# 0411tony/Yue

Hardware: AMD Instinct MI355X
Metric: BPR triplet-updates/sec at k=128 (S-round semantics, user rows sequential; the reference's exact sequential semantics: secondary.exact) (higher is better)
Workload: dtype f32

## Files before the change

yue_amd/csrc/bpr_host.hip:

```cpp
#include "host_common.hpp"

#include "train_kernels.hpp"
#include "round_kernels.hpp"

using yue_host::fail;
using yue_host::kr_of;
using yue_host::with_kr;
static_assert(yue::kNllSlots == yue_host::kNllSlotsHost && yue::kHeaderSlack == yue_host::kHeaderSlackHost &&
              yue::kMetaStageMax == (uint32_t)yue_host::kMetaStageMaxHost, "host_common.hpp mirrors these");

namespace {

yue::TrainArgs make_args(yue_ctx *c, double lr, double regU, double regI) {
    yue::TrainArgs a{};
    a.P = c->P.p; a.Q = c->Q.p; a.dP = c->dP.p; a.dQ = c->dQ.p;
    a.stage = c->Q.p ? c->Q.p + (size_t)c->n * c->k : nullptr;
    a.ev_u = c->ev_u.p; a.ev_i = c->ev_i.p; a.ev_j = c->ev_j.p;
    a.indptr = c->indptr.p; a.indices = c->indices.p;
    a.nll_slots = c->scal.p;
    a.m = c->m; a.n = c->n; a.k = c->k;
    a.lr = lr;
    a.ru = (float)(lr * regU);
    a.ri = (float)(lr * regI);
    a.neg_lo = 0; a.neg_range = (int32_t)c->n;
// ... 351 lines not shown
    if (!c || !c->have_factors) return fail(YUE_ERR_ARG, "yue_bpr_replay: no factors uploaded");
    if (T < 0 || (T > 0 && (!u || !i || !j))) return fail(YUE_ERR_ARG, "yue_bpr_replay: bad triplet arrays");
    HIPCHK(hipSetDevice(c->device));
    if (!c->opt_replay_levels) {
        int rc = upload_triplets(c, u, i, j, T, false);
        if (rc) return rc;
        if ((rc = zero_scalars(c))) return rc;
        if ((rc = yue_host::chain_stream(c, T, lr, regU, regI))) return rc;
        return read_scalars(c, nll_out, nullptr, nullptr);
    }
    std::vector<int32_t> lastP((size_t)c->m, 0), lastQ((size_t)c->n, 0), lvl((size_t)T);
    int32_t nlev = 0;
    for (int64_t t = 0; t < T; ++t) {
        if (u[t] < 0 || u[t] >= c->m || i[t] < 0 || i[t] >= c->n || j[t] >= c->n) return fail(YUE_ERR_ARG, "triplet " + std::to_string(t) + " out of range");
        if (j[t] < 0) { lvl[(size_t)t] = 0; continue; }
        if (i[t] == j[t]) return fail(YUE_ERR_ARG, "triplet " + std::to_string(t) + ": i == j");
        int32_t l = std::max(lastP[(size_t)u[t]], std::max(lastQ[(size_t)i[t]], lastQ[(size_t)j[t]])) + 1;
        lvl[(size_t)t] = l;
        lastP[(size_t)u[t]] = lastQ[(size_t)i[t]] = lastQ[(size_t)j[t]] = l;
        nlev = std::max(nlev, l);
    }
    std::vector<int64_t> lptr((size_t)nlev + 2, 0);
    for (int64_t t = 0; t < T; ++t) if (lvl[(size_t)t] > 0) lptr[(size_t)lvl[(size_t)t] + 1]++;
    for (int32_t l = 1; l <= nlev; ++l) lptr[(size_t)l + 1] += lptr[(size_t)l];
    const int64_t Tv = lptr[(size_t)nlev + 1];
    std::vector<int32_t> pu((size_t)std::max<int64_t>(Tv, 1)), pi((size_t)std::max<int64_t>(Tv, 1)), pj((size_t)std::max<int64_t>(Tv, 1));
    {
        std::vector<int64_t> cur(lptr.begin(), lptr.end());
        for (int64_t t = 0; t < T; ++t) {
            const int32_t l = lvl[(size_t)t];
            if (l == 0) continue;
            const int64_t o = cur[(size_t)l]++;
            pu[(size_t)o] = u[t]; pi[(size_t)o] = i[t]; pj[(size_t)o] = j[t];
        }
    }
    int rc = upload_triplets(c, pu.data(), pi.data(), pj.data(), Tv, true);
    if (rc) return rc;
    yue::TrainArgs a = make_args(c, lr, regU, regI);
    a.ev_u = c->xu.p; a.ev_i = c->xi.p; a.ev_j = c->xj.p;
    if ((rc = zero_scalars(c))) return rc;
    c->replay_levels = nlev;
    for (int32_t l = 1; l <= nlev; ++l) {
        const int64_t e0 = lptr[(size_t)l], e1 = lptr[(size_t)l + 1];
        if (e1 > e0) launch_level(c, a, e0, e1);
    }
    HIPCHK(hipGetLastError());
    return read_scalars(c, nll_out, nullptr, nullptr);
}

int yue_bpr_rounds(yue_ctx *c, const int32_t *u, const int32_t *i, const int32_t *j, const int64_t *round_ptr, int64_t n_rounds,
                   double lr, double regU, double regI, double *nll_out) {
    if (!c || !c->have_factors) return fail(YUE_ERR_ARG, "yue_bpr_rounds: no factors uploaded");
    if (!round_ptr || n_rounds < 0) return fail(YUE_ERR_ARG, "yue_bpr_rounds: bad round_ptr");
    HIPCHK(hipSetDevice(c->device));
    const int64_t T = round_ptr[n_rounds];
    if (round_ptr[0] != 0) return fail(YUE_ERR_ARG, "yue_bpr_rounds: round_ptr[0] must be 0");
    for (int64_t r = 0; r < n_rounds; ++r) if (round_ptr[r + 1] < round_ptr[r]) return fail(YUE_ERR_ARG, "yue_bpr_rounds: round_ptr must be non-decreasing");
    if (c->m * (int64_t)c->k * 4 >= (1ll << 31)) {
        const int tpw = tpw_of(c, false);
        for (int64_t r = 0; r < n_rounds; ++r)
            for (int64_t b = round_ptr[r]; b < round_ptr[r + 1]; b += tpw) {
                int32_t lo = u[b], hi = u[b];
                for (int64_t t = b; t < std::min(round_ptr[r + 1], b + tpw); ++t) { lo = std::min(lo, u[t]); hi = std::max(hi, u[t]); }
                if ((int64_t)(hi - lo) * c->k * 4 >= (1ll << 31)) return fail(YUE_ERR_ARG, "yue_bpr_rounds: users of neighbouring triplets are more than 2 GiB of factor rows apart; group the triplets by user");
            }
    }
    int rc = upload_triplets(c, u, i, j, T, true);
    if (rc) return rc;
    yue::TrainArgs a = make_args(c, lr, regU, regI);
    a.ev_u = c->xu.p; a.ev_i = c->xi.p; a.ev_j = c->xj.p;
    if ((rc = zero_scalars(c))) return rc;
    std::vector<int64_t> bounds(round_ptr, round_ptr + n_rounds + 1);
    if ((rc = run_rounds(c, a, bounds, 1, [](int64_t) { return YUE_OK; }))) { reset_round_state(c); return rc; }
    HIPCHK(hipGetLastError());
    return read_scalars(c, nll_out, nullptr, nullptr);
}

int yue_cune_steps(yue_ctx *c, const int32_t *u, const int32_t *i, const int32_t *k, const int32_t *j, int64_t T,
                   double s, double lr, double regU, double regI, double *loss_out) {
    if (!c || !c->have_factors) return fail(YUE_ERR_ARG, "yue_cune_steps: no factors uploaded");
    if (T < 0 || (T > 0 && (!u || !i || !k || !j || !loss_out)) || !(s > 0.0)) return fail(YUE_ERR_ARG, "yue_cune_steps: bad argument");
    if (T == 0) return YUE_OK;
    HIPCHK(hipSetDevice(c->device));
    for (int64_t t = 0; t < T; ++t) {
        if (u[t] < 0 || u[t] >= c->m || i[t] < 0 || i[t] >= c->n || j[t] < 0 || j[t] >= c->n || k[t] >= c->n) return fail(YUE_ERR_ARG, "yue_cune_steps: step " + std::to_string(t) + " out of range");
        if (i[t] == j[t] || k[t] == i[t]) return fail(YUE_ERR_ARG, "yue_cune_steps: step " + std::to_string(t) + ": i must differ from k and from j (k == j is allowed, as in the reference)");
    }
    int rc = upload_triplets(c, u, i, j, T, true);
    if (rc) return rc;
    HIPCHK(c->xk.resize(T)); HIPCHK(c->x_loss.resize(T));
    HIPCHK(hipMemcpyAsync(c->xk.p, k, T * sizeof(int32_t), hipMemcpyHostToDevice, c->stream));
    yue::CuneArgs a{};
    a.P = c->P.p; a.Q = c->Q.p; a.k = c->k; a.u = c->xu.p; a.i = c->xi.p; a.kk = c->xk.p; a.j = c->xj.p; a.T = T;
    a.inv_s = 1.0 / s; a.inv_s32 = (float)(1.0 / s); a.lr = lr;
    a.ru = (float)(lr * regU); a.ri = (float)(lr * regI);
    a.loss_out = c->x_loss.p;
    with_kr(c->k, [&](auto kr) { hipLaunchKernelGGL(yue::k_cune_steps<kr()>, dim3(1), dim3(64), 0, c->stream, a); });
    HIPCHK(hipGetLastError());
    HIPCHK(hipMemcpyAsync(loss_out, c->x_loss.p, T * sizeof(double), hipMemcpyDeviceToHost, c->stream));
    HIPCHK(hipStreamSynchronize(c->stream));
    return YUE_OK;
}

int yue_adam_reset(yue_ctx *c) {
    if (!c || !c->have_factors) return fail(YUE_ERR_ARG, "yue_adam_reset: no factors uploaded");
    HIPCHK(hipSetDevice(c->device));
    const size_t mk = (size_t)c->m * c->k, nk = (size_t)c->n * c->k;
    HIPCHK(c->aU_m.resize(mk)); HIPCHK(c->aU_v.resize(mk)); HIPCHK(c->aV_m.resize(nk)); HIPCHK(c->aV_v.resize(nk));
    HIPCHK(hipMemsetAsync(c->aU_m.p, 0, mk * sizeof(float), c->stream)); HIPCHK(hipMemsetAsync(c->aU_v.p, 0, mk * sizeof(float), c->stream));
    HIPCHK(hipMemsetAsync(c->aV_m.p, 0, nk * sizeof(float), c->stream)); HIPCHK(hipMemsetAsync(c->aV_v.p, 0, nk * sizeof(float), c->stream));
    HIPCHK(hipMemsetAsync(c->dP.p, 0, mk * sizeof(float), c->stream)); HIPCHK(hipMemsetAsync(c->dQ.p, 0, nk * sizeof(float), c->stream));
    c->adam_m = c->m; c->adam_n = c->n; c->adam_k = c->k;
    return YUE_OK;
}

int yue_adam_get_moments(yue_ctx *c, float *mU, float *vU, float *mV, float *vV) {
    if (!c || !c->have_factors || c->adam_m != c->m || c->adam_n != c->n || c->adam_k != c->k)
        return fail(YUE_ERR_ARG, "yue_adam_get_moments: no Adam state for the uploaded factors");
    HIPCHK(hipSetDevice(c->device));
    HIPCHK(hipStreamSynchronize(c->stream));
    const size_t mk = (size_t)c->m * c->k * sizeof(float), nk = (size_t)c->n * c->k * sizeof(float);
    if (mU) HIPCHK(hipMemcpy(mU, c->aU_m.p, mk, hipMemcpyDeviceToHost));
    if (vU) HIPCHK(hipMemcpy(vU, c->aU_v.p, mk, hipMemcpyDeviceToHost));
    if (mV) HIPCHK(hipMemcpy(mV, c->aV_m.p, nk, hipMemcpyDeviceToHost));
    if (vV) HIPCHK(hipMemcpy(vV, c->aV_v.p, nk, hipMemcpyDeviceToHost));
    return YUE_OK;
}

int yue_adam_step(yue_ctx *c, const int32_t *u, const int32_t *i, const int32_t *j, int64_t T, double lr, double reg, int64_t step, double *loss_out) {
    if (!c || !c->have_factors) return fail(YUE_ERR_ARG, "yue_adam_step: no factors uploaded");
    if (T <= 0 || !u || !i || !j || step < 1) return fail(YUE_ERR_ARG, "yue_adam_step: bad argument (T > 0, step >= 1)");
    HIPCHK(hipSetDevice(c->device));
    if (c->adam_m != c->m || c->adam_n != c->n || c->adam_k != c->k) { const int rc0 = yue_adam_reset(c); if (rc0) return rc0; }
    for (int64_t t = 0; t < T; ++t)
        if (u[t] < 0 || u[t] >= c->m || i[t] < 0 || i[t] >= c->n || j[t] < 0 || j[t] >= c->n) return fail(YUE_ERR_ARG, "yue_adam_step: triplet " + std::to_string(t) + " out of range");
    int rc = upload_triplets(c, u, i, j, T, true);
    if (rc) return rc;
    if ((rc = zero_scalars(c))) return rc;
    yue::MbArgs a{};
    a.U = c->P.p; a.V = c->Q.p; a.gU = c->dP.p; a.gV = c->dQ.p; a.k = c->k; a.u = c->xu.p; a.i = c->xi.p; a.j = c->xj.p; a.T = T;
    a.reg = (float)reg; a.loss_slots = c->scal.p;
    const dim3 grid((unsigned)(((T + 31) / 32 + 3) / 4));
    with_kr(c->k, [&](auto kr) { hipLaunchKernelGGL(yue::k_mb_grad<kr()>, grid, dim3(256), 0, c->stream, a); });
    if ((rc = yue_host::adam_apply(c, lr, step))) return rc;
    return read_scalars(c, loss_out, nullptr, nullptr);
}

int yue_sample_negatives(yue_ctx *c, uint64_t seed, uint32_t epoch, int32_t *j_out) {
    if (!c || !c->have_inter || !j_out) return fail(YUE_ERR_ARG, "yue_sample_negatives: no interactions uploaded");
    HIPCHK(hipSetDevice(c->device));
    yue::TrainArgs a = make_args(c, 0, 0, 0);
    a.seed = seed; a.epoch = epoch;
    if (c->E > 0) {
        hipLaunchKernelGGL(yue::k_sample, dim3((unsigned)((c->E + 255) / 256)), dim3(256), 0, c->stream, a, c->E);
        HIPCHK(hipGetLastError());
        HIPCHK(hipMemcpyAsync(j_out, c->ev_j.p, c->E * sizeof(int32_t), hipMemcpyDeviceToHost, c->stream));
    }
    HIPCHK(hipStreamSynchronize(c->stream));
    return YUE_OK;
}

int yue_sumsq(yue_ctx *c, double *sp, double *sq) {
    if (!c || !c->have_factors) return fail(YUE_ERR_ARG, "yue_sumsq: no factors uploaded");
    HIPCHK(hipSetDevice(c->device));
    int rc = sumsq_async(c);
    if (rc) return rc;
    double h[2];
    HIPCHK(hipMemcpyAsync(h, c->scal.p + yue::kNllSlots + 1, sizeof h, hipMemcpyDeviceToHost, c->stream));
    HIPCHK(hipStreamSynchronize(c->stream));
    if (sp) *sp = h[0];
    if (sq) *sq = h[1];
    return YUE_OK;
}

int yue_bpr_epoch(yue_ctx *c, uint64_t seed, uint32_t epoch, int64_t round_events, double lr, double regU, double regI,
                  double *nll_out, double *sumsqP_out, double *sumsqQ_out) {
    if (!c || !c->have_factors || !c->have_inter) return fail(YUE_ERR_ARG, "yue_bpr_epoch: upload factors and interactions first");
    if (round_events < 0) return fail(YUE_ERR_ARG, "yue_bpr_epoch: round_events must be positive (or 0 for the device's default)");
    HIPCHK(hipSetDevice(c->device));
    yue::TrainArgs a = make_args(c, lr, regU, regI);
    a.seed = seed + 0x632BE59BD9B4E019ull * (uint64_t)c->rank;
    a.epoch = epoch;
    int rc = zero_scalars(c);
    if (rc) return rc;
    const int64_t E = c->E;
    if (E > 0) hipLaunchKernelGGL(yue::k_sample, dim3((unsigned)((E + 255) / 256)), dim3(256), 0, c->stream, a, E);
    if (c->opt_epoch_exact) {
        if (yue_host::on_communicator(c) && c->nranks > 1) return fail(YUE_ERR_ARG, "yue_bpr_epoch: option epoch_exact runs on one GPU (the sequential order spans all item shards)");
        if ((rc = yue_host::chain_epoch(c, lr, regU, regI))) return rc;
        if ((rc = sumsq_async(c))) return rc;
        return read_scalars(c, nll_out, sumsqP_out, sumsqQ_out);
    }
    std::vector<int64_t> bounds;
    double tot[2] = {(double)E, (double)c->n};
    if (yue_host::on_communicator(c)) {
        if ((rc = yue_allreduce_f64(c, tot, 2))) return rc;
        if ((rc = zero_scalars(c))) return rc;
    }
    const double etot = tot[0];
    if (round_events == 0 && (rc = default_round_events(c, tot[1] / c->nranks, &round_events))) return rc;
    int64_t ub = 1, group = 1;
    if ((rc = yue_epoch_plan(c->m, c->k, round_events, etot, c->nranks, &ub, &group, nullptr))) return rc;
    if (!yue_host::on_communicator(c)) group = std::max<int64_t>(1, (c->m + ub - 1) / ub);
    else group = std::max<int64_t>(1, ((int64_t)c->opt_comm_group_mb << 20) / std::max<int64_t>(1, ub * c->k * 4));
    std::vector<int64_t> ublock;
    for (int64_t u0 = 0; u0 < c->m; u0 += ub) { ublock.push_back(u0); bounds.push_back(c->h_ev_ptr[(size_t)u0]); }
    ublock.push_back(c->m); bounds.push_back(E);
    const int64_t R = (int64_t)ublock.size() - 1;
    const bool seq_user = !yue_host::on_communicator(c) && c->opt_round_user_seq && meta_path_fits(c);
    if (seq_user) {
        HIPCHK(c->d_ev_ptr.resize((size_t)c->m + 1));
        if (!c->d_ev_ptr_valid) {
            HIPCHK(hipMemcpyAsync(c->d_ev_ptr.p, c->h_ev_ptr.data(), ((size_t)c->m + 1) * sizeof(int64_t), hipMemcpyHostToDevice, c->stream));
            c->d_ev_ptr_valid = true;
        }
        HIPCHK(c->margins.resize((size_t)std::max<int64_t>(E, 1)));
    }
    c->psq_in_rounds = seq_user && c->all_users_have_events && E > 0;
    if (c->psq_in_rounds) {
        HIPCHK(c->psq_slots.resize((size_t)yue::kNllSlots));
        HIPCHK(hipMemsetAsync(c->psq_slots.p, 0, (size_t)yue::kNllSlots * sizeof(double), c->stream));
    }
    c->last_round_user_seq = 0;
    auto after = [&](int64_t r) -> int {
        if (seq_user && !c->bigq) { c->last_round_user_seq = 1; return YUE_OK; }
        if ((r + 1) % group != 0 && r + 1 != R) return YUE_OK;
        const int64_t g_first = ublock[(size_t)(r - (r % group))], g_last = ublock[(size_t)r + 1];
        const int64_t first = g_first * c->k, count = (g_last - g_first) * c->k;
        const dim3 grid((unsigned)std::min<int64_t>(4096, (count + 255) / 256));
        if (!yue_host::on_communicator(c)) {
            hipLaunchKernelGGL(yue::k_apply_range, grid, dim3(256), 0, c->stream, c->P.p, c->dP.p, first, count);
            return YUE_OK;
        }
        HIPCHK(hipEventRecord(c->ev_rounds, c->stream));
        HIPCHK(hipStreamWaitEvent(c->comm_stream, c->ev_rounds, 0));
        c->comm_collectives += 1;
        c->comm_bytes += (double)count * sizeof(float);
        if (const int rcr = yue_host::reduce_user_block(c, first, count, c->comm_stream)) return rcr;
        hipLaunchKernelGGL(yue::k_apply_range, grid, dim3(256), 0, c->comm_stream, c->P.p, c->dP.p, first, count);
        return YUE_OK;
    };
    c->comm_collectives = 0; c->comm_bytes = 0.0; c->comm_wait_ms = 0.0;
    if ((rc = run_rounds(c, a, bounds, 0, after, meta_path_fits(c), seq_user ? &ublock : nullptr))) { reset_round_state(c); return rc; }
    if (c->last_round_user_seq && E > 0)
        hipLaunchKernelGGL(yue::k_loss_margins, dim3(2048), dim3(256), 0, c->stream, c->margins.p, c->ev_j.p, E, c->scal.p);
    const bool psq_done = c->psq_in_rounds && c->last_round_user_seq;
    c->psq_in_rounds = false;
    if (yue_host::on_communicator(c)) {
        HIPCHK(hipEventRecord(c->ev_t_rounds, c->stream));
        HIPCHK(hipEventRecord(c->ev_t_comm, c->comm_stream));
    }
    HIPCHK(hipEventRecord(c->ev_comm, c->comm_stream));
    HIPCHK(hipStreamWaitEvent(c->stream, c->ev_comm, 0));
    c->comm_compute_waits = 1;
    HIPCHK(hipGetLastError());
    if ((rc = sumsq_async(c, psq_done ? c->psq_slots.p : nullptr))) return rc;
    if ((rc = read_scalars(c, nll_out, sumsqP_out, sumsqQ_out))) return rc;
    if (yue_host::on_communicator(c)) {
        float ms = 0.f;
        HIPCHK(hipEventSynchronize(c->ev_t_comm));
        HIPCHK(hipEventElapsedTime(&ms, c->ev_t_rounds, c->ev_t_comm));
        c->comm_wait_ms = ms > 0.f ? ms : 0.0;
    }
    return YUE_OK;
}

int yue_epoch_plan(int64_t m, int k, int64_t round_events, double events_total, int nranks,
                   int64_t *user_block, int64_t *blocks_per_group, int64_t *n_blocks) {
    if (m <= 0 || k <= 0 || round_events <= 0 || nranks < 1 || !(events_total >= 0.0)) return fail(YUE_ERR_ARG, "yue_epoch_plan: bad argument");
    const double per_user = events_total / (double)nranks / (double)m;
    const int64_t ub = std::max<int64_t>(1, (int64_t)std::floor((double)round_events / std::max(per_user, 1e-9) + 0.5));
    if (user_block) *user_block = ub;
    if (blocks_per_group) *blocks_per_group = std::max<int64_t>(1, (8ll << 20) / std::max<int64_t>(1, ub * k * 4));
    if (n_blocks) *n_blocks = (m + ub - 1) / ub;
    return YUE_OK;
}

int yue_default_round_events(yue_ctx *c, int64_t *out) {
    if (!c || !c->have_factors || !out) return fail(YUE_ERR_ARG, "yue_default_round_events: upload factors first (the value depends on k)");
    HIPCHK(hipSetDevice(c->device));
    double n_rows = (double)c->n;
    if (yue_host::on_communicator(c)) {
        const int rc = yue_allreduce_f64(c, &n_rows, 1);
        if (rc) return rc;
        n_rows /= c->nranks;
    }
    return default_round_events(c, n_rows, out);
}

int yue_set_kernel_timing(yue_ctx *c, int stride) {
    if (!c || stride < 0) return fail(YUE_ERR_ARG, "yue_set_kernel_timing: bad argument");
    c->timing_stride = stride;
    c->ev_used = 0;
    return YUE_OK;
}

int yue_get_kernel_timing(yue_ctx *c, double *total_ms, int64_t *launches, int64_t *triplets) {
    if (!c) return fail(YUE_ERR_ARG, "null context");
    HIPCHK(hipSetDevice(c->device));
    HIPCHK(hipStreamSynchronize(c->stream));
    double tot = 0.0;
    int64_t trip = 0, nl = 0;
    for (size_t t = 0; t < c->ev_used; ++t) {
        float ms = 0.f;
        HIPCHK(hipEventElapsedTime(&ms, c->ev_pool[t].first, c->ev_pool[t].second));
        tot += ms;
        trip += c->ev_triplets[t];
        nl += c->ev_launches[t];
    }
    if (total_ms) *total_ms = tot;
    if (launches) *launches = nl;
    if (triplets) *triplets = trip;
    c->ev_used = 0;
    return YUE_OK;
}

#ifdef YUE_STAMPS
int yue_debug_get_stamps(yue_ctx *c, unsigned long long *out, int64_t max_waves, int64_t *n_waves) {
    HIPCHK(hipStreamSynchronize(c->stream));
    const int64_t w = std::min(max_waves, c->stamp_waves);
    if (w > 0) HIPCHK(hipMemcpy(out, c->stamps.p, (size_t)w * 64, hipMemcpyDeviceToHost));
    *n_waves = w;
    return YUE_OK;
}
#endif

}
```

yue_amd/csrc/round_kernels.hpp:

```cpp
#pragma once
#include "train_kernels.hpp"

#ifdef YUE_ABL_NO_HOT
#define YUE_M_HOT(val, rs, vo, so) asm volatile("" :: "v"(val))
#else
#define YUE_M_HOT(val, rs, vo, so) YUE_BATOMIC(val, rs, vo, so)
#endif
#ifdef YUE_ABL_NO_DP
#define YUE_M_DP(val, rs, vo, so) asm volatile("" :: "v"(val))
#else
#define YUE_M_DP(val, rs, vo, so) YUE_BATOMIC(val, rs, vo, so)
#endif

#define YUE_BLOAD_NT(rs, vo, so) __builtin_bit_cast(float, __builtin_amdgcn_raw_buffer_load_b32((rs), (vo), (so), 2))
#if defined(YUE_EXP_LOAD_CACHED)
#define YUE_M_LOAD_J(rs, vo, so) YUE_BLOAD(rs, vo, so)
#define YUE_M_LOAD_I(rs, vo, so) YUE_BLOAD(rs, vo, so)
#elif defined(YUE_EXP_LOAD_NT)
#define YUE_M_LOAD_J(rs, vo, so) YUE_BLOAD_NT(rs, vo, so)
#define YUE_M_LOAD_I(rs, vo, so) YUE_BLOAD_NT(rs, vo, so)
#else
#define YUE_M_LOAD_J(rs, vo, so) YUE_BLOAD_NT(rs, vo, so)
#define YUE_M_LOAD_I(rs, vo, so) YUE_BLOAD(rs, vo, so)
#endif
// ... 347 lines not shown
                    }
                }
            } else {
            if (!hot_i) {
#pragma unroll
                for (int r = 0; r < KR; ++r) YUE_BSTORE(full_i ? o[r].qi2 : o[r].qi2 - qi[t][r], rsQ, vo[r], wi);
            } else {
#pragma unroll
                for (int r = 0; r < KR; ++r) YUE_M_HOT(o[r].qi2 - qi[t][r], rsdQ, vo[r], oi[t]);
            }
            if (!hot_j) {
#pragma unroll
                for (int r = 0; r < KR; ++r) YUE_BSTORE(full_j ? o[r].qj2 : o[r].qj2 - qj[t][r], rsQ, vo[r], wj);
            } else {
#pragma unroll
                for (int r = 0; r < KR; ++r) YUE_M_HOT(o[r].qj2 - qj[t][r], rsdQ, vo[r], oj[t]);
            }
            }
        }
        const bool exists = base + t < ra.e_end;
        const bool last = exists && ((t == TPW - 1) || base + t + 1 >= ra.e_end || ru_[t + 1 < TPW ? t + 1 : t] != ru_[t]);
        if (last) {
            if (run_ok) {
#pragma unroll
                for (int r = 0; r < KR; ++r) YUE_M_DP(dp[r], rsdP, vo[r], ou[t]);
            }
#pragma unroll
            for (int r = 0; r < KR; ++r) dp[r] = 0.0f;
            run_ok = false;
        }
        __builtin_amdgcn_sched_barrier(0);
    }
    YUE_STAMP(4, ""); YUE_STAMP(5, ""); YUE_STAMP(6, "");
#pragma unroll
    for (int off = 1; off < TPW; off <<= 1) nll += __shfl_xor(nll, off);
    if (lane == 0 && nll != 0.0) atomicAdd(a.nll_slots + (wave & (kNllSlots - 1)), nll);
    YUE_STAMP(7, "s_waitcnt vmcnt(0)");
}

struct RoundUArgs {
    int64_t u_begin, u_end;
    const int64_t *ev_ptr;
    int64_t e_begin, e_end;
    int staged;
    float *margins;
    double *psq_slots;
};

template <int KR, bool FAST>
__global__ void __launch_bounds__(256) k_round_u(TrainArgs a, RoundUArgs ra, const int32_t *__restrict__ evi, const int32_t *__restrict__ evj,
                                                 const uint32_t *__restrict__ mti, const uint32_t *__restrict__ mtj) {
    const int lane = threadIdx.x & 63;
    const int64_t wave = (int64_t)blockIdx.x * 4 + __builtin_amdgcn_readfirstlane((int)(threadIdx.x >> 6));
    const int64_t u = ra.u_begin + wave;
    if (u >= ra.u_end) return;
    const int64_t e0 = ra.ev_ptr[u], e1 = ra.ev_ptr[u + 1];
    if (e1 <= e0) return;
    const unsigned k = (unsigned)a.k;
    const unsigned row_bytes = k * 4u;
    unsigned vo[KR];
#pragma unroll
    for (int r = 0; r < KR; ++r) { const unsigned e = 64u * r + lane; vo[r] = e < k ? e * 4u : kOobOffset; }
    const uint64_t qbytes = (uint64_t)a.n * row_bytes;
    const int qrec = (int)(qbytes < 0x7fffffffull ? qbytes : 0x7fffffffull);
    const unsigned stage0 = (unsigned)a.n * row_bytes;
    const uint64_t qsbytes = qbytes + (ra.staged ? 2ull * (uint64_t)(ra.e_end - ra.e_begin) * row_bytes : 0ull);
    const int qsrec = (int)(qsbytes < 0x7fffffffull ? qsbytes : 0x7fffffffull);
    const auto rsQ = __builtin_amdgcn_make_buffer_rsrc(a.Q, 0, qsrec, kRsrcFlags);
    const auto rsdQ = __builtin_amdgcn_make_buffer_rsrc(a.dQ, 0, qrec, kRsrcFlags);
    float *prow = a.P + (uint64_t)u * k;
    float p[KR];
#pragma unroll
    for (int r = 0; r < KR; ++r) { const unsigned e = 64u * r + lane; p[r] = e < k ? prow[e] : 0.0f; }
    const float lrf = (float)a.lr;
    const unsigned len = (unsigned)(e1 - e0 < 0x7fffffff ? e1 - e0 : 0x7fffffff);
    for (unsigned seg = 0; seg < len; seg += 64u) {
        int hI, hJ;
        uint32_t hMI, hMJ;
        {
            const bool ex = seg + (unsigned)lane < len;
            const int64_t e = e0 + seg + (ex ? lane : 0);
            hI = evi[e]; hJ = evj[e]; hMI = mti[e]; hMJ = mtj[e];
            if (!ex) { hI = 0; hJ = -1; hMI = 0u; hMJ = 0u; }
        }
        const unsigned seg_len = len - seg < 64u ? len - seg : 64u;
        float xs = 0.0f;
        auto gather = [&](float (&qi)[KR], float (&qj)[KR], unsigned t) {
            const int ti = __builtin_amdgcn_readlane(hI, t), tj = __builtin_amdgcn_readlane(hJ, t);
            const unsigned oi = (unsigned)ti * row_bytes, oj = (unsigned)(tj < 0 ? 0 : tj) * row_bytes;
#pragma unroll
            for (int r = 0; r < KR; ++r) { qi[r] = YUE_M_LOAD_I(rsQ, vo[r], oi); qj[r] = YUE_M_LOAD_J(rsQ, vo[r], oj); }
        };
        auto step = [&](const float (&qi)[KR], const float (&qj)[KR], unsigned t) {
            const int tj = __builtin_amdgcn_readlane(hJ, t);
            if (tj < 0) return;
            const int ti = __builtin_amdgcn_readlane(hI, t);
            const uint32_t mi = (uint32_t)__builtin_amdgcn_readlane((int)hMI, t), mj = (uint32_t)__builtin_amdgcn_readlane((int)hMJ, t);
            float ai = 0.0f, aj = 0.0f;
#pragma unroll
            for (int r = 0; r < KR; ++r) { const float a1 = p[r] * qi[r]; ai = ai + a1; const float a2 = p[r] * qj[r]; aj = aj + a2; }
            const float x = wave_sum(ai) - wave_sum(aj);
            const float c = FAST ? chain_coef_fast(x, lrf) : (float)(a.lr * (1.0 - chain_sigmoid(x)));
            xs = (unsigned)lane == t ? x : xs;
            const unsigned cli = meta_kind(mi), clj = meta_kind(mj);
            const bool uniq_i = cli == kMetaUnique, uniq_j = clj == kMetaUnique;
            const bool full_i = uniq_i || meta_first(mi), full_j = uniq_j || meta_first(mj);
            const unsigned oi = (unsigned)ti * row_bytes, oj = (unsigned)tj * row_bytes;
            const unsigned wi = uniq_i ? oi : stage0 + meta_slot(mi) * row_bytes;
            const unsigned wj = uniq_j ? oj : stage0 + meta_slot(mj) * row_bytes;
            Elem o[KR];
#pragma unroll
            for (int r = 0; r < KR; ++r) { o[r] = bpr_elem(p[r], qi[r], qj[r], c, a.ru, a.ri); p[r] = o[r].p2; }
            if (cli != kMetaHot) {
#pragma unroll
                for (int r = 0; r < KR; ++r) YUE_BSTORE(full_i ? o[r].qi2 : o[r].qi2 - qi[r], rsQ, vo[r], wi);
            } else {
#pragma unroll
                for (int r = 0; r < KR; ++r) YUE_M_HOT(o[r].qi2 - qi[r], rsdQ, vo[r], oi);
            }
            if (clj != kMetaHot) {
#pragma unroll
                for (int r = 0; r < KR; ++r) YUE_BSTORE(full_j ? o[r].qj2 : o[r].qj2 - qj[r], rsQ, vo[r], wj);
            } else {
#pragma unroll
                for (int r = 0; r < KR; ++r) YUE_M_HOT(o[r].qj2 - qj[r], rsdQ, vo[r], oj);
            }
        };
        constexpr int D = KR == 1 ? 8 : 4;
        float qi[D][KR], qj[D][KR];
#pragma unroll
        for (int s_ = 0; s_ < D; ++s_) gather(qi[s_], qj[s_], (unsigned)s_);
        for (unsigned t = 0; t < seg_len; t += D) {
#pragma unroll
            for (int s_ = 0; s_ < D; ++s_) {
                step(qi[s_], qj[s_], t + s_);
                gather(qi[s_], qj[s_], (t + s_ + D) & 63u);
            }
        }
        if ((unsigned)lane < seg_len) ra.margins[e0 + seg + lane] = xs;
    }
#pragma unroll
    for (int r = 0; r < KR; ++r) { const unsigned e = 64u * r + lane; if (e < k) prow[e] = p[r]; }
    if (ra.psq_slots) {
        double s = 0.0;
#pragma unroll
        for (int r = 0; r < KR; ++r) { const unsigned e = 64u * r + lane; const float sq = p[r] * p[r]; if (e < k) s += (double)sq; }
#pragma unroll
        for (int off = 1; off < 64; off <<= 1) s += __shfl_xor(s, off);
        if (lane == 0) atomicAdd(ra.psq_slots + (u & (kNllSlots - 1)), s);
    }
}

__global__ void __launch_bounds__(256) k_loss_margins(const float *__restrict__ x, const int32_t *__restrict__ evj, int64_t E, double *nll_slots) {
    double nl = 0.0;
    const int64_t stride = (int64_t)gridDim.x * blockDim.x;
    for (int64_t e = (int64_t)blockIdx.x * blockDim.x + threadIdx.x; e < E; e += stride)
        if (evj[e] >= 0) nl += -log(chain_sigmoid(x[e]));
#pragma unroll
    for (int off = 1; off < 64; off <<= 1) nl += __shfl_xor(nl, off);
    if ((threadIdx.x & 63) == 0 && nl != 0.0) atomicAdd(nll_slots + ((blockIdx.x * 4 + (threadIdx.x >> 6)) & (kNllSlots - 1)), nl);
}

struct FoldArgs {
    const uint2 *fold;
    const unsigned long long *round_rows;
    float *Q, *dQ;
    const float *stage;
    int k;
    uint32_t capacity;
};

template <int KR, int EPG>
__device__ __forceinline__ void fold_group(const FoldArgs &f, int lane, unsigned k, uint32_t nact, const uint2 (&ent)[4]) {
    float st[EPG][4][KR];
    unsigned el[KR];
    bool big = false;
#pragma unroll
    for (int r = 0; r < KR; ++r) el[r] = min(64u * r + lane, k - 1u);
#pragma unroll
    for (int sl = 0; sl < EPG; ++sl) {
        if ((uint32_t)sl >= nact) continue;
        const uint32_t c = fold_count(ent[sl].y);
        const bool hot = c == 0u;
        const float *src = hot ? f.dQ + (uint64_t)ent[sl].x * k : f.stage + (uint64_t)fold_block(ent[sl].y) * k;
#pragma unroll
        for (int r = 0; r < KR; ++r) st[sl][0][r] = YUE_FOLD_LD(src + el[r]);
        if (hot) {
            const float *row = f.Q + (uint64_t)ent[sl].x * k;
#pragma unroll
            for (int r = 0; r < KR; ++r) st[sl][1][r] = YUE_FOLD_LDROW(row + el[r]);
        } else {
#pragma unroll
            for (int r = 0; r < KR; ++r) st[sl][1][r] = YUE_FOLD_LD(src + (uint64_t)k + el[r]);
        }
        if (c > 2u) {
#pragma unroll
            for (unsigned q = 2; q < 4; ++q)
#pragma unroll
                for (int r = 0; r < KR; ++r) st[sl][q][r] = YUE_FOLD_LD(src + (uint64_t)(q < c ? q : 0u) * k + el[r]);
        }
        big = big || c > 4u;
    }
#pragma unroll
    for (int sl = 0; sl < EPG; ++sl) {
        if ((uint32_t)sl >= nact) continue;
        const uint32_t c = fold_count(ent[sl].y);
        const bool hot = c == 0u;
        float *row = f.Q + (uint64_t)ent[sl].x * k;
        float *dr = f.dQ + (uint64_t)ent[sl].x * k;
#pragma unroll
        for (int r = 0; r < KR; ++r) {
            const unsigned e = 64u * r + lane;
            float acc = st[sl][1][r];
#pragma unroll
            for (unsigned q = 2; q < 4; ++q) { const float v = q < c ? st[sl][q][r] : 0.0f; acc = acc + v; }
            st[sl][1][r] = acc;
            if (c <= 4u && e < k) {
                row[e] = st[sl][0][r] + acc;
                if (hot) dr[e] = 0.0f;
            }
        }
    }
    if (big) {
#pragma unroll
        for (int sl = 0; sl < EPG; ++sl) {
            if ((uint32_t)sl >= nact) continue;
            const uint32_t c = fold_count(ent[sl].y);
            if (c <= 4u) continue;
            const float *src = f.stage + (uint64_t)fold_block(ent[sl].y) * k;
            float *row = f.Q + (uint64_t)ent[sl].x * k;
            float acc[KR];
#pragma unroll
            for (int r = 0; r < KR; ++r) acc[r] = st[sl][1][r];
            constexpr unsigned STEP = KR == 1 ? 8u : 4u;
            for (uint32_t q0 = 4u; q0 < c; q0 += STEP) {
                float v[STEP][KR];
#pragma unroll
                for (unsigned q = 0; q < STEP; ++q)
#pragma unroll
                    for (int r = 0; r < KR; ++r) v[q][r] = YUE_FOLD_LD(src + (uint64_t)(q0 + q < c ? q0 + q : q0) * k + el[r]);
#pragma unroll
                for (unsigned q = 0; q < STEP; ++q)
#pragma unroll
                    for (int r = 0; r < KR; ++r) acc[r] = acc[r] + (q0 + q < c ? v[q][r] : 0.0f);
            }
#pragma unroll
            for (int r = 0; r < KR; ++r) { const unsigned e = 64u * r + lane; if (e < k) row[e] = st[sl][0][r] + acc[r]; }
        }
    }
}

template <int KR>
__global__ void __launch_bounds__(256) k_round_fold(FoldArgs f) {
    constexpr int EPG = KR == 4 ? 2 : 4;
    const int lane = threadIdx.x & 63;
    const uint32_t wave = blockIdx.x * 4u + (uint32_t)__builtin_amdgcn_readfirstlane((int)(threadIdx.x >> 6));
    const uint32_t nwaves = gridDim.x * 4u;
    const unsigned k = (unsigned)f.k;
    const uint32_t b0 = wave * EPG;
    uint2 ent[4];
    typedef uint32_t u32x8 __attribute__((ext_vector_type(8)));
    u32x8 ev;
    unsigned long long cntw;
    const bool spec = b0 + 4u <= f.capacity;
    const uint2 *first = f.fold + (spec ? b0 : 0u);
    asm volatile("s_load_dwordx8 %0, %2, 0x0\n\ts_load_dwordx2 %1, %3, 0x0\n\ts_waitcnt lgkmcnt(0)"
                 : "=&s"(ev), "=&s"(cntw) : "s"(first), "s"(f.round_rows) : "memory");
    const uint32_t cnt = (uint32_t)(cntw >> 32);
    ent[0] = make_uint2(ev[0], ev[1]); ent[1] = make_uint2(ev[2], ev[3]); ent[2] = make_uint2(ev[4], ev[5]); ent[3] = make_uint2(ev[6], ev[7]);
    if (b0 < cnt) {
        if (!spec) {
#pragma unroll
            for (int sl = 0; sl < EPG; ++sl) ent[sl] = f.fold[b0 + sl < cnt ? b0 + sl : b0];
        }
        fold_group<KR, EPG>(f, lane, k, min((uint32_t)EPG, cnt - b0), ent);
    }
    for (uint32_t b = b0 + nwaves * EPG; b < cnt; b += nwaves * EPG) {
#pragma unroll
        for (int sl = 0; sl < EPG; ++sl) ent[sl] = f.fold[b + sl < cnt ? b + sl : b];
        fold_group<KR, EPG>(f, lane, k, min((uint32_t)EPG, cnt - b), ent);
    }
}

}
```

yue_amd/csrc/train_kernels.hpp:

```cpp
#pragma once
#include "bpr_device.hpp"

namespace yue {

__global__ void __launch_bounds__(256) k_sample(TrainArgs a, int64_t E) {
    int64_t e = (int64_t)blockIdx.x * blockDim.x + threadIdx.x;
    if (e < E) a.ev_j[e] = sample_negative(a, a.ev_u[e], e);
}

template <int KR>
__global__ void __launch_bounds__(256) k_bpr_level(TrainArgs a, int64_t e_begin, int64_t e_end, int tpw) {
    const int lane = threadIdx.x & 63;
    const int64_t wave = (int64_t)blockIdx.x * (blockDim.x >> 6) + (threadIdx.x >> 6);
    const int64_t base = e_begin + wave * tpw;
    if (base >= e_end) return;
    const int cnt = (int)((e_end - base) < (int64_t)tpw ? (e_end - base) : (int64_t)tpw);
    int u = 0, i = 0, j = 0;
    if (lane < cnt) { u = a.ev_u[base + lane]; i = a.ev_i[base + lane]; j = a.ev_j[base + lane]; }
    const int k = a.k;
    double nll = 0.0;
    for (int t = 0; t < cnt; ++t) {
        const int64_t tu = __builtin_amdgcn_readlane(u, t);
        const int64_t ti = __builtin_amdgcn_readlane(i, t);
        const int64_t tj = __builtin_amdgcn_readlane(j, t);
        float p[KR], qi[KR], qj[KR];
#pragma unroll
        for (int r = 0; r < KR; ++r) {
            const int e = 64 * r + lane;
            p[r] = e < k ? a.P[tu * k + e] : 0.0f;
            qi[r] = e < k ? a.Q[ti * k + e] : 0.0f;
            qj[r] = e < k ? a.Q[tj * k + e] : 0.0f;
        }
        float ai = 0.0f, aj = 0.0f;
#pragma unroll
        for (int r = 0; r < KR; ++r) { const float a1 = p[r] * qi[r]; ai = ai + a1; const float a2 = p[r] * qj[r]; aj = aj + a2; }
        const float x = wave_sum(ai) - wave_sum(aj);
        const double s = 1.0 / (1.0 + exp(-(double)x));
        const float c = (float)(a.lr * (1.0 - s));
        nll += -log(s);
#pragma unroll
        for (int r = 0; r < KR; ++r) {
            const int e = 64 * r + lane;
            const Elem o = bpr_elem(p[r], qi[r], qj[r], c, a.ru, a.ri);
            if (e < k) { a.P[tu * k + e] = o.p2; a.Q[ti * k + e] = o.qi2; a.Q[tj * k + e] = o.qj2; }
        }
    }
    if (lane == 0) atomicAdd(a.nll_slots + (wave & (kNllSlots - 1)), nll);
}

struct MbArgs {
    const float *U, *V;
    float *gU, *gV;
    int k;
    const int32_t *u, *i, *j;
    int64_t T;
    float reg;
    double *loss_slots;
};

template <int KR>
__global__ void __launch_bounds__(256) k_mb_grad(MbArgs a) {
    constexpr int CH = 32;
    const int lane = threadIdx.x & 63;
    const int64_t wave = (int64_t)blockIdx.x * 4 + (threadIdx.x >> 6);
    const int64_t t0 = wave * CH;
    if (t0 >= a.T) return;
    const int64_t t1 = t0 + CH < a.T ? t0 + CH : a.T;
    const int k = a.k;
    float pu[KR], vi[KR], gu[KR], gvi[KR];
    int64_t cu = -1, ci = -1;
    float dui = 0.0f, su = 0.0f, si = 0.0f;
    double loss = 0.0;
    auto flush = [&]() {
        if (cu < 0) return;
#pragma unroll
        for (int r = 0; r < KR; ++r) {
            const int e = 64 * r + lane;
            if (e < k) { atomicAdd(a.gU + cu * k + e, gu[r]); atomicAdd(a.gV + ci * k + e, gvi[r]); }
        }
    };
    for (int64_t t = t0; t < t1; ++t) {
        const int64_t u = a.u[t], i = a.i[t], j = a.j[t];
        if (u != cu || i != ci) {
            flush();
            cu = u; ci = i;
            float d = 0.0f, q1 = 0.0f, q2 = 0.0f;
#pragma unroll
            for (int r = 0; r < KR; ++r) {
                const int e = 64 * r + lane;
                pu[r] = e < k ? a.U[u * k + e] : 0.0f;
                vi[r] = e < k ? a.V[i * k + e] : 0.0f;
                gu[r] = 0.0f; gvi[r] = 0.0f;
                d = __builtin_fmaf(pu[r], vi[r], d); q1 = __builtin_fmaf(pu[r], pu[r], q1); q2 = __builtin_fmaf(vi[r], vi[r], q2);
            }
            dui = wave_sum(d); su = wave_sum(q1); si = wave_sum(q2);
        }
        float vn[KR];
        float d = 0.0f, q3 = 0.0f;
#pragma unroll
        for (int r = 0; r < KR; ++r) {
            const int e = 64 * r + lane;
            vn[r] = e < k ? a.V[j * k + e] : 0.0f;
            d = __builtin_fmaf(pu[r], vn[r], d); q3 = __builtin_fmaf(vn[r], vn[r], q3);
        }
        const float err = dui - wave_sum(d);
        const float sn = wave_sum(q3);
        const float ax = __builtin_fabsf(err);
        loss += (double)(fmaxf(-err, 0.0f) + log1pf(expf(-ax)));
        loss += (double)(0.5f * a.reg * (su + si + sn));
        const float g = -1.0f / (1.0f + expf(err));
#pragma unroll
        for (int r = 0; r < KR; ++r) {
            const int e = 64 * r + lane;
            gu[r] = gu[r] + (g * (vi[r] - vn[r]) + a.reg * pu[r]);
            gvi[r] = gvi[r] + (g * pu[r] + a.reg * vi[r]);
            if (e < k) atomicAdd(a.gV + j * k + e, -g * pu[r] + a.reg * vn[r]);
        }
    }
    flush();
    if (lane == 0) atomicAdd(a.loss_slots + (wave & (kNllSlots - 1)), loss);
}

__global__ void __launch_bounds__(256) k_adam(float *var, float *m, float *v, float *grad, int64_t count, float lr_t, float beta1, float beta2, float eps) {
    const int64_t stride = (int64_t)gridDim.x * blockDim.x;
    for (int64_t t = (int64_t)blockIdx.x * blockDim.x + threadIdx.x; t < count; t += stride) {
        const float g = grad[t];
        const float m1 = beta1 * m[t] + (1.0f - beta1) * g;
        const float v1 = beta2 * v[t] + ((1.0f - beta2) * g) * g;
        m[t] = m1; v[t] = v1;
        var[t] = var[t] - lr_t * m1 / (__builtin_sqrtf(v1) + eps);
        if (g != 0.0f) grad[t] = 0.0f;
    }
}

struct CuneArgs {
    float *P, *Q;
    int k;
    const int32_t *u, *i, *kk, *j;
    int64_t T;
    double inv_s, lr;
    float inv_s32;
    float ru, ri;
    double *loss_out;
};

template <int KR>
__global__ void __launch_bounds__(64) k_cune_steps(CuneArgs a) {
    const int lane = threadIdx.x;
    const int k = a.k;
    auto dot = [&](const float (&x)[KR], const float (&y)[KR]) {
        float acc = 0.0f;
#pragma unroll
        for (int r = 0; r < KR; ++r) { const float m = x[r] * y[r]; acc = acc + m; }
        return wave_sum(acc);
    };
    auto sig = [](double x) { return 1.0 / (1.0 + exp(-x)); };
    for (int64_t t = 0; t < a.T; ++t) {
        const int64_t u = a.u[t], i = a.i[t], kq = a.kk[t], j = a.j[t];
        float p[KR], qi[KR], qk[KR], qj[KR];
#pragma unroll
// ... 352 lines not shown
```

Before: 1.833 billion.

## Stage user interaction windows in LDS for negative sampling; batch loss logs

The negative-sampling kernel now handles 1024 events per block. It loads the contiguous CSR span of positives for those users into shared memory and binary-searches there instead of in global memory, falling back to the old per-event path when the span exceeds 4096 entries. Separately, the loss-margin reduction accumulates a product of (1+exp(-x)) using frexp mantissa/exponent tracking and takes one log per thread instead of one per event, with a second pass for extreme margins. This relies on events being sorted by user for the window to be compact, and changes floating-point rounding of the loss sum.

```diff
diff --git a/yue_amd/csrc/bpr_host.hip b/yue_amd/csrc/bpr_host.hip
--- a/yue_amd/csrc/bpr_host.hip
+++ b/yue_amd/csrc/bpr_host.hip
@@ -527,7 +527,7 @@
     yue::TrainArgs a = make_args(c, 0, 0, 0);
     a.seed = seed; a.epoch = epoch;
     if (c->E > 0) {
-        hipLaunchKernelGGL(yue::k_sample, dim3((unsigned)((c->E + 255) / 256)), dim3(256), 0, c->stream, a, c->E);
+        hipLaunchKernelGGL(yue::k_sample, dim3((unsigned)((c->E + yue::kSampleEvents - 1) / yue::kSampleEvents)), dim3(256), 0, c->stream, a, c->E);
         HIPCHK(hipGetLastError());
         HIPCHK(hipMemcpyAsync(j_out, c->ev_j.p, c->E * sizeof(int32_t), hipMemcpyDeviceToHost, c->stream));
     }
@@ -559,7 +559,7 @@
     int rc = zero_scalars(c);
     if (rc) return rc;
     const int64_t E = c->E;
-    if (E > 0) hipLaunchKernelGGL(yue::k_sample, dim3((unsigned)((E + 255) / 256)), dim3(256), 0, c->stream, a, E);
+    if (E > 0) hipLaunchKernelGGL(yue::k_sample, dim3((unsigned)((E + yue::kSampleEvents - 1) / yue::kSampleEvents)), dim3(256), 0, c->stream, a, E);
     if (c->opt_epoch_exact) {
         if (yue_host::on_communicator(c) && c->nranks > 1) return fail(YUE_ERR_ARG, "yue_bpr_epoch: option epoch_exact runs on one GPU (the sequential order spans all item shards)");
         if ((rc = yue_host::chain_epoch(c, lr, regU, regI))) return rc;
diff --git a/yue_amd/csrc/round_kernels.hpp b/yue_amd/csrc/round_kernels.hpp
--- a/yue_amd/csrc/round_kernels.hpp
+++ b/yue_amd/csrc/round_kernels.hpp
@@ -523,10 +523,27 @@
 }
 
 __global__ void __launch_bounds__(256) k_loss_margins(const float *__restrict__ x, const int32_t *__restrict__ evj, int64_t E, double *nll_slots) {
-    double nl = 0.0;
-    const int64_t stride = (int64_t)gridDim.x * blockDim.x;
-    for (int64_t e = (int64_t)blockIdx.x * blockDim.x + threadIdx.x; e < E; e += stride)
-        if (evj[e] >= 0) nl += -log(chain_sigmoid(x[e]));
+    double mant = 1.0, far = 0.0;
+    int ex = 0;
+    bool any_far = false;
+    const int64_t stride = (int64_t)gridDim.x * blockDim.x, first = (int64_t)blockIdx.x * blockDim.x + threadIdx.x;
+    for (int64_t e = first; e < E; e += stride)
+        if (evj[e] >= 0) {
+            const double xd = (double)x[e];
+            if (__builtin_fabs(xd) <= 700.0) {
+                int s;
+                mant = __builtin_frexp(mant * (1.0 + chain_exp(-xd)), &s);
+                ex += s;
+            } else any_far = true;
+        }
+    if (any_far)
+        for (int64_t e = first; e < E; e += stride)
+            if (evj[e] >= 0) {
+                const double xd = (double)x[e];
+                if (!(__builtin_fabs(xd) <= 700.0)) far += -log(1.0 / (1.0 + exp(-xd)));
+            }
+    if (mant < 7.07106781186547524401e-01) { mant *= 2.0; ex -= 1; }
+    double nl = far + (log(mant) + (double)ex * 6.93147180559945286227e-01);
 #pragma unroll
     for (int off = 1; off < 64; off <<= 1) nl += __shfl_xor(nl, off);
     if ((threadIdx.x & 63) == 0 && nl != 0.0) atomicAdd(nll_slots + ((blockIdx.x * 4 + (threadIdx.x >> 6)) & (kNllSlots - 1)), nl);
diff --git a/yue_amd/csrc/train_kernels.hpp b/yue_amd/csrc/train_kernels.hpp
--- a/yue_amd/csrc/train_kernels.hpp
+++ b/yue_amd/csrc/train_kernels.hpp
@@ -3,9 +3,62 @@
 
 namespace yue {
 
+constexpr int kSampleWindow = 4096;
+constexpr int kSampleEvents = 1024;
+
 __global__ void __launch_bounds__(256) k_sample(TrainArgs a, int64_t E) {
-    int64_t e = (int64_t)blockIdx.x * blockDim.x + threadIdx.x;
-    if (e < E) a.ev_j[e] = sample_negative(a, a.ev_u[e], e);
+    constexpr int EPT = kSampleEvents / 256;
+    __shared__ int32_t win[kSampleWindow];
+    __shared__ int64_t wbound[2];
+    const int tid = threadIdx.x;
+    const int64_t e0 = (int64_t)blockIdx.x * kSampleEvents;
+    const int n_ev = (int)(E - e0 < (int64_t)kSampleEvents ? E - e0 : (int64_t)kSampleEvents);
+    int32_t u[EPT];
+    int64_t lo[EPT], hi[EPT];
+#pragma unroll
+    for (int q = 0; q < EPT; ++q) u[q] = a.ev_u[e0 + (q * 256 + tid < n_ev ? q * 256 + tid : n_ev - 1)];
+#pragma unroll
+    for (int q = 0; q < EPT; ++q) { lo[q] = a.indptr[u[q]]; hi[q] = a.indptr[(int64_t)u[q] + 1]; }
+#pragma unroll
+    for (int q = 0; q < EPT; ++q) {
+        if (q * 256 + tid == 0) wbound[0] = lo[q];
+        if (q * 256 + tid == n_ev - 1) wbound[1] = hi[q];
+    }
+    __syncthreads();
+    const int64_t w_lo = wbound[0], w_hi = wbound[1];
+    if (w_hi - w_lo > (int64_t)kSampleWindow) {
+#pragma unroll
+        for (int q = 0; q < EPT; ++q)
+            if (q * 256 + tid < n_ev) a.ev_j[e0 + q * 256 + tid] = sample_negative(a, u[q], e0 + q * 256 + tid);
+        return;
+    }
+    const int w = (int)(w_hi - w_lo);
+    for (int t0 = 0; t0 < w; t0 += 256 * EPT) {
+        int32_t v[EPT];
+#pragma unroll
+        for (int q = 0; q < EPT; ++q) { const int t = t0 + q * 256 + tid; v[q] = a.indices[w_lo + (t < w ? t : w - 1)]; }
+#pragma unroll
+        for (int q = 0; q < EPT; ++q) { const int t = t0 + q * 256 + tid; if (t < w) win[t] = v[q]; }
+    }
+    __syncthreads();
+#pragma unroll
+    for (int q = 0; q < EPT; ++q) {
+        if (q * 256 + tid >= n_ev) continue;
+        const int64_t e = e0 + q * 256 + tid;
+        const int r_lo = (int)(lo[q] - w_lo), r_hi = (int)(hi[q] - w_lo);
+        int32_t out = -1;
+        for (uint32_t t = 0; t < (uint32_t)kMaxAttempts; ++t) {
+            const int32_t c = ctr_draw(a.seed, a.epoch, (uint64_t)e, t, a.neg_lo, a.neg_range);
+            int base = r_lo, len = r_hi - r_lo;
+            while (len > 1) {
+                const int half = len >> 1;
+                base = win[base + half] <= c ? base + half : base;
+                len -= half;
+            }
+            if (len == 0 || win[base] != c) { out = c; break; }
+        }
+        a.ev_j[e] = out;
+    }
 }
 
 template <int KR>
```

Result: faster. 1.864 billion, median of 6 (+1.7%).
